# bioinformatics-centre/BayesTyper

Measured on AMD Instinct MI355X. Metric: variant-cluster Gibbs iterations/sec + k-mer matches/sec at 1/2/4/8 MI355X, higher is better.
Workload: dtype f64 log-probabilities over u8 k-mer counts (Gibbs); u64/u8 integer (k-mer matching)

## Files before the change

bayestyper_amd/csrc/bt_gibbs.hip:

```cpp
#ifndef BT_SWEEP_OUTLINE
#define BT_SWEEP_INLINE
#endif
#include "bt_gibbs_kernel.hpp"
#include "bt_internal.hpp"

#include <algorithm>
#include <atomic>
#include <chrono>
#include <cmath>
#include <cstring>
#include <map>
#include <memory>
#include <numeric>

using namespace bt;

namespace bt {
hipError_t launch_gibbs_simple_kernel(unsigned grid, uint32_t lds, hipStream_t st, const TileDesc *tiles, uint8_t *pool, const GParams *P, int op, uint32_t a0, uint32_t a1,
                                      unsigned long long *hist, TraceCfg tr, const uint32_t *tile_list);
hipError_t prepare_gibbs_simple_kernel(int max_lds);
hipError_t launch_gibbs_hot_kernel(unsigned grid, unsigned block, uint32_t lds, hipStream_t st, const TileDesc *tiles, uint8_t *pool, const GParams *P, int op, uint32_t a0, uint32_t a1,
                                   unsigned long long *hist, TraceCfg tr, const uint32_t *tile_list);
hipError_t prepare_gibbs_hot_kernel(int max_lds);
hipError_t occupancy_gibbs_hot_kernel(int *blocks_per_cu, int block, uint32_t lds);
// ... 664 lines not shown
    const bool fork = g->classes.size() > 1;
    if (fork) BT_HIP(hipEventRecord(g->ev_fork, g->ctx->stream));
    const char *order_env = getenv("BT_GIBBS_ORDER");
    const bool hot_first = order_env && std::strcmp(order_env, "hot_first") == 0 && (op == OP_RUN || op == OP_SWEEP);
    const bool ordered = (op == OP_RUN || op == OP_SWEEP) && !getenv("BT_GIBBS_UNORDERED_START");
    const bt_gibbs::LaunchClass *prev = nullptr;
    for (auto &c : g->classes) {
        hipStream_t st = c.stream ? c.stream : g->ctx->stream;
        if (c.stream) BT_HIP(hipStreamWaitEvent(st, g->ev_fork, 0));
        if (ordered && prev) BT_HIP(hipStreamWaitEvent(st, prev->ready, 0));
        if (hot_first && !c.stream)
            for (auto &o : g->classes)
                if (o.stream) BT_HIP(hipStreamWaitEvent(st, o.done, 0));
        if (op == OP_SWEEP && g->prefill_armed && c.num_prefill) {
            const unsigned threads = (uint64_t)c.num_prefill * g->S >= 4096 ? 64u : 256u;
            hipLaunchKernelGGL(ucache_prefill_kernel, dim3(c.num_prefill, g->S), dim3(threads), 0, st, (const TileDesc *)g->d_tiles, g->d_pool, (const GParams *)g->d_params,
                               (const PrefillItem *)c.d_prefill);
            BT_CHECK_LAUNCH();
        }
        if (ordered) {
            BT_HIP(hipEventRecord(c.ready, st));
            prev = &c;
        }
        if (op == OP_NOISE && (size_t)g->S * 1024 <= kHotBudget && !g->noise_in_gibbs_kernel) {
            const unsigned grid = (unsigned)std::min<size_t>(c.tiles.size(), (size_t)g->ctx->num_cu * 4);
            hipLaunchKernelGGL(gibbs_noise_kernel, dim3(grid), dim3(LANES * c.split), (size_t)g->S * 1024, st, (const TileDesc *)g->d_tiles, g->d_pool, (const GParams *)g->d_params, a0, hist,
                               (const uint32_t *)c.d_tiles, (uint32_t)c.tiles.size());
        } else if (c.simple && (op == OP_RUN || op == OP_SWEEP || op == OP_INIT_CHAIN))
            BT_HIP(launch_gibbs_simple_kernel((unsigned)c.tiles.size(), c.lds, st, g->d_tiles, g->d_pool, g->d_params, op, a0, a1, hist, tr, (const uint32_t *)c.d_tiles));
        else if (c.single && (op == OP_RUN || op == OP_SWEEP || op == OP_INIT_CHAIN))
            BT_HIP(launch_gibbs_single_kernel(c.pack_wgs, LANES * c.pack_waves, c.pack_lds, st, g->d_tiles, g->d_pool, g->d_params, op, a0, a1, hist, tr, (const uint32_t *)c.d_pack));
        else if (c.hot && (op == OP_RUN || op == OP_SWEEP || op == OP_INIT_CHAIN))
            BT_HIP(launch_gibbs_hot_kernel(c.pack_wgs, LANES * c.pack_waves, c.pack_lds, st, g->d_tiles, g->d_pool, g->d_params, op, a0, a1, hist, tr, (const uint32_t *)c.d_pack));
        else
            hipLaunchKernelGGL(gibbs_kernel, dim3((unsigned)c.tiles.size()), dim3(LANES * c.split), c.lds, st, g->d_tiles, g->d_pool, g->d_params, op, a0, a1, hist, tr,
                               (const uint32_t *)c.d_tiles);
        BT_CHECK_LAUNCH();
        if (wide && c.num_fill) {
            hipLaunchKernelGGL(nan_fill_kernel, dim3(c.num_fill), dim3(256), 0, st, g->d_pool, (const FillChunk *)c.d_fill);
            BT_CHECK_LAUNCH();
        }
        if (c.stream) BT_HIP(hipEventRecord(c.done, st));
    }
    for (auto &c : g->classes)
        if (c.stream) BT_HIP(hipStreamWaitEvent(g->ctx->stream, c.done, 0));
    g->prefill_armed = wide;
    return BT_OK;
}

inline uint64_t align_up(uint64_t x, uint64_t a) { return (x + a - 1) / a * a; }
inline uint32_t tile_lds_bytes(const TileDesc &d) { return d.lds_all ? d.hot_bytes * d.nvm : d.hot_bytes; }
constexpr uint32_t kMinTileWidth = 4;
constexpr uint32_t kLightLds = 24576;
const uint32_t kClassLds[] = {16384, 32768, 0xFFFFFFFFu};

const uint32_t kElemSize[A_COUNT] = {
     1,  1,  1,  1,  4,  4,  2,  4,  2,  4,  4,  4,  2,
     1,  4,  4,  4,  2,  4,  4,  4,  4,  4,  4,
     4,  1,
     4,  8,  8,  4,  4,  4,  4,  1,  2,  8,  4,  1,
     4,  4,  4,  4,  4,  4,  8,  4,  8,  2,  8,
     8,  4,  8,  1,  4,  4,  8,  1,  1,  8,  4,  8,  4,  1,  4,  8,  4,
     4,  1,  8,  4,  4,  4,  1,  1,  1,  1,  4,  2,  4,  8,  8,  4,  2,  1,  4,  4,  4,  1,  1,  1,  1,  4,  4};

}

extern "C" {

struct bt_gibbs_source {
    bt_ctx *ctx = nullptr;
    uint32_t S = 0, G = 0, C = 0;
    std::vector<ClusterDims> cd;
    std::vector<GroupDims> gd;
    BuildBatch dev{};
    std::vector<void *> allocs;
    uint64_t device_bytes = 0, flat_bytes = 0;
    bool uploaded = false;
};

static int validate_batch(const bt_gibbs_batch *B) {
    const uint32_t G = B->num_groups, C = B->num_clusters;
    if (G == 0 || C == 0) return fail("bt_gibbs_create: empty batch");
    if (B->group_cluster_off[G] != C) return fail("bt_gibbs_create: group_cluster_off[G] != num_clusters");
    {
        auto monotone = [](const uint32_t *off, uint64_t n) {
            for (uint64_t i = 0; i < n; ++i)
                if (off[i + 1] < off[i]) return false;
            return true;
        };
        if (B->group_cluster_off[0] != 0 || !monotone(B->group_cluster_off, G) || !monotone(B->group_source_off, G) || !monotone(B->edge_off, C) || !monotone(B->kmer_off, C) ||
            !monotone(B->unique_off, C) || !monotone(B->multi_off, C) || !monotone(B->nestdep_off, C) || !monotone(B->kv_off, B->kmer_off[C]) ||
            !monotone(B->nestdep_var_off, B->nestdep_off[C]))
            return fail("bt_gibbs_create: an offset array of the batch is not monotone");
        uint64_t hap_at = 0, var_at = 0, hv_at = 0;
        for (uint32_t gi = 0; gi < G; ++gi) {
            const uint32_t c0 = B->group_cluster_off[gi], c1 = B->group_cluster_off[gi + 1], nv = c1 - c0;
            if (nv == 0) return fail("bt_gibbs_create: group without clusters");
            for (uint32_t i = B->group_source_off[gi]; i < B->group_source_off[gi + 1]; ++i)
                if (B->group_sources[i] >= nv) return fail("bt_gibbs_create: source vertex outside its group");
            for (uint32_t c = c0; c < c1; ++c) {
                const uint32_t H = B->num_haplotypes[c], V = B->num_variants[c], K = B->kmer_off[c + 1] - B->kmer_off[c];
                for (uint32_t i = B->edge_off[c]; i < B->edge_off[c + 1]; ++i)
                    if (B->edges[i] >= nv) return fail("bt_gibbs_create: edge target outside its group");
                for (uint32_t i = B->unique_off[c]; i < B->unique_off[c + 1]; ++i)
                    if (B->unique_idx[i] >= K) return fail("bt_gibbs_create: unique k-mer index outside its cluster");
                for (uint32_t i = B->multi_off[c]; i < B->multi_off[c + 1]; ++i)
// ... 237 lines not shown
            return _rc;          \
        }                        \
    } while (0)
#define BT_TRYHIP(x)                                                     \
    do {                                                                 \
        hipError_t _e = (x);                                             \
        if (_e != hipSuccess) {                                          \
            bt_gibbs_destroy(g);                                         \
            return fail(std::string(#x) + ": " + hipGetErrorString(_e)); \
        }                                                                \
    } while (0)

    g->h_A.assign(C, 0);
    uint64_t flat_sel = 0;
    for (uint32_t c = 0; c < C; ++c) {
        g->h_A[c] = cd[c].A;
        flat_sel += (uint64_t)cd[c].K * cd[c].H + (uint64_t)cd[c].K * (S + 11ull) + (uint64_t)cd[c].nnz * (2 + 4 * ((cd[c].H + 31) / 32)) + ((uint64_t)cd[c].nu + cd[c].nm) * 4 +
                    (uint64_t)cd[c].H * cd[c].V * 2 + (uint64_t)cd[c].H * 4 + (uint64_t)cd[c].hn * 4;
    }

    const bool timing = getenv("BT_GIBBS_DEBUG") != nullptr;
    auto t_prev = std::chrono::steady_clock::now();
    std::string t_text;
    auto lap = [&](const char *what) {
        if (!timing) return;
        const auto now = std::chrono::steady_clock::now();
        char buf[96];
        snprintf(buf, sizeof buf, " %s %.1f ms;", what, std::chrono::duration<double, std::milli>(now - t_prev).count());
        t_text += buf;
        t_prev = now;
    };
    struct GShape {
        uint32_t nv, Hmax, Kmax, g;
    };
    std::vector<GShape> shapes(G);
    for (uint32_t gi = 0; gi < G; ++gi) {
        GShape s{gd[gi].nv, 0, 0, gi};
        for (uint32_t c = gd[gi].c0; c < gd[gi].c0 + gd[gi].nv; ++c) {
            s.Hmax = std::max(s.Hmax, cd[c].H);
            s.Kmax = std::max(s.Kmax, cd[c].K);
        }
        shapes[gi] = s;
    }
    std::stable_sort(shapes.begin(), shapes.end(), [](const GShape &a, const GShape &b) {
        if (a.nv != b.nv) return a.nv > b.nv;
        if (a.Hmax != b.Hmax) return a.Hmax > b.Hmax;
        return a.Kmax > b.Kmax;
    });
    std::vector<uint32_t> tile_start, blk_first, blk_last;
    std::vector<TilePlan> plans;
    uint64_t pool = 0;
    uint32_t ntiles = 0;
    uint32_t noise_level = 0;
    auto plan_tiles = [&](uint32_t relax) {
    tile_start.clear();
    pool = 0;
    const uint64_t dense_limit = relax >= 4 ? (64ull << 20) : (256ull << 20);
    {
        const uint32_t tail_h = getenv("BT_GIBBS_TAIL_H") ? (uint32_t)atoi(getenv("BT_GIBBS_TAIL_H")) : 16u;
        uint32_t n_x = 0;
        while (n_x < G && (shapes[n_x].nv > 1 || shapes[n_x].Hmax >= tail_h)) ++n_x;
        uint32_t n_y = n_x;
        while (n_y < G && shapes[n_y].Hmax >= 6) ++n_y;
        uint32_t width_x = kMinTileWidth, width_y = 16;
        const bool noise_widths = params->noise_seeding && !getenv("BT_GIBBS_NO_NOISE_WIDTHS");
        uint32_t width_z3 = LANES;
        if (noise_widths) {
            if (noise_level == 0) width_y = 8, width_z3 = 32;
            else if (noise_level == 1) width_y = 16, width_z3 = 32;
            else width_y = 16, width_z3 = LANES;
        }
        width_x = std::min<uint32_t>(LANES, width_x << relax);
        width_y = std::min<uint32_t>(LANES, width_y << relax);
        if (const char *e = getenv("BT_GIBBS_TAIL_WIDTH")) {
            const int v = atoi(e);
            if (v == 1 || v == 2 || v == 4 || v == 8 || v == 16 || v == 32 || v == 64) width_x = (uint32_t)v;
        }
        if (const char *e = getenv("BT_GIBBS_MID_WIDTH")) {
            const int v = atoi(e);
            if (v == 4 || v == 8 || v == 16 || v == 32 || v == 64) width_y = (uint32_t)v;
        }
        auto hashed = [&](uint32_t i) { return (uint64_t)S * ((uint64_t)shapes[i].Hmax * (shapes[i].Hmax + 1) / 2 + shapes[i].Hmax) > 65536; };
        uint32_t n_w = 0;
        for (uint32_t i = 0; i < n_x; ++i) n_w += hashed(i) ? 1u : 0u;
        uint32_t width_w = 1;
        while (width_w < width_x && (uint64_t)n_w > (uint64_t)width_w * (4 * 256)) width_w *= 2;
        if (const char *e = getenv("BT_GIBBS_HUGE_WIDTH")) {
            const int v = atoi(e);
            if (v == 1 || v == 2 || v == 4 || v == 8 || v == 16) width_w = (uint32_t)v;
        }
        width_w = std::min<uint32_t>(width_x, width_w << relax);
        uint32_t at = 0;
        while (at < n_x) {
            const bool hw = hashed(at);
            uint32_t run_end = at;
            while (run_end < n_x && hashed(run_end) == hw) ++run_end;
            const uint32_t w = hw ? width_w : width_x;
            while (at < run_end) {
                tile_start.push_back(at);
                at += std::min<uint32_t>(w, run_end - at);
            }
        }
        while (at < n_y) {
            tile_start.push_back(at);
            at += std::min<uint32_t>(width_y, n_y - at);
        }
        uint32_t n_z = n_y, n_z3 = n_y;
        if (noise_widths) {
            while (n_z < G && shapes[n_z].Hmax >= 4) ++n_z;
// ... 215 lines not shown
        for (int a = 0; a < A_COUNT; ++a) {
            off = align_up(off, 256);
            d.off[a] = off;
            off += len[a] * tile_w * kElemSize[a];
            if (a == A_PLOIDY) in_bytes = align_up(off, 256);
        }
        {
            for (int a = 0; a < A_COUNT; ++a) d.hoff[a] = NOHOT;
            const int hot_arrs[] = {A_SC, A_DIP, A_NESTPL, A_NESTN, A_KSCUPD, A_MGEN, A_PEND, A_PENDDIP, A_PENDVALID, A_EVN, A_FREQ, A_LOGF, A_OBS, A_NZ, A_NZLIST,
                                    A_UNEXT, A_ZHDR, A_ZBKT, A_PHDR, A_PBKT, A_KSCTMP, A_CUM, A_RING, A_FNDSAVED, A_UCACHE};
            d.lds_stride = 1;
            while (d.lds_stride < d.num_lanes) d.lds_stride *= 2;
            uint64_t ho = 0;
            bool want_simple = d.nvm == 1 && d.Hm == 2 && d.NMm == 0 && d.cache_mode == 0 && d.lds_stride == LANES && !getenv("BT_GIBBS_NO_SIMPLE") && !getenv("BT_GIBBS_NO_SIMPLE_KERNEL");
            for (uint32_t l = 0; l < d.num_lanes && want_simple; ++l) want_simple = cd[gd[shapes[tile_start[ti] + l].g].c0].H == 2;
            const uint64_t skip_mask = getenv("BT_GIBBS_HOT_SKIP") ? strtoull(getenv("BT_GIBBS_HOT_SKIP"), nullptr, 0) : 0ull;
            int hot_i = -1;
            for (int a : hot_arrs) {
                ++hot_i;
                if ((skip_mask >> hot_i) & 1ull) continue;
                if (a == A_MGEN && d.NMm == 0) continue;
                if (a == A_KSCTMP) continue;
                if (a == A_CUM && d.D2m * d.teams > 16) continue;
                if (want_simple && a != A_RING) continue;
                if (a == A_UCACHE && !(d.cache_mode == 0 && d.uc_width == 0 && d.nvm == 1 && (uint64_t)d.cache_entries * 8 <= 160)) continue;
                const uint64_t per_vertex = len[a] / nv;
                d.hoff[a] = (uint32_t)ho;
                ho = align_up(ho + per_vertex * d.lds_stride * kElemSize[a], 16);
            }
            d.sblk = 0;
            if (want_simple) {
                d.sblk = (uint32_t)ho;
                ho = align_up(ho + (uint64_t)3 * S * LANES * 4, 16);
            }
            d.hot_bytes = (uint32_t)std::min<uint64_t>(ho, 0xFFFFFFFFu);
            const uint64_t hot_budget = getenv("BT_GIBBS_HOT_BUDGET") ? strtoull(getenv("BT_GIBBS_HOT_BUDGET"), nullptr, 0) : kHotBudget;
            d.lds_all = d.nvm > 1 && ho * d.nvm <= hot_budget && !getenv("BT_GIBBS_NO_LDS_ALL") ? 1u : 0u;
            if (ho > hot_budget || (d.nvm > 1 && !d.lds_all && hot_budget < kHotBudget) || (d.nvm > 1 && getenv("BT_GIBBS_NOHOT_MULTI"))) {
                for (int a = 0; a < A_COUNT; ++a) d.hoff[a] = NOHOT;
                d.hot_bytes = 0;
                d.lds_all = 0;
            }
        }
        d.split = d.Hm < 6 ? 1u : (tile_lds_bytes(d) > kLightLds ? 2u : 4u);
        if (const char *e = getenv("BT_GIBBS_SPLIT")) {
            const int v = atoi(e);
            if (v == 1 || v == 2 || v == 4 || v == 8) d.split = (uint32_t)v;
        }
        d.copies = 1;
        if (d.lds_stride <= 32 && !getenv("BT_GIBBS_NO_COPIES")) {
            d.split = 1;
            d.copies = 64u / d.lds_stride;
        }
        {
            bool simple = d.nvm == 1 && d.Hm == 2 && d.NMm == 0 && d.cache_mode == 0 && d.copies == 1 && d.split == 1 && d.hot_bytes != 0 && !getenv("BT_GIBBS_NO_SIMPLE");
            for (uint32_t l = 0; l < d.num_lanes && simple; ++l) simple = cd[gd[shapes[tile_start[ti] + l].g].c0].H == 2;
            simple = simple && d.sblk != 0 && d.hoff[A_RING] != NOHOT && d.hoff[A_SC] == NOHOT;
            d.simple = simple ? 1u : 0u;
        }
        d.logged = d.nvm == 1 && d.NMm == 0 && !getenv("BT_GIBBS_NO_LOG") ? 1u : 0u;
        d.prio = (d.copies > 1 || d.num_lanes < LANES / 2) && !getenv("BT_GIBBS_NO_PRIO") ? 1u : 0u;
        d.base = ti == blk_first[ti] ? pool : plans[blk_first[ti]].d.base;
        if (ti == 0 && getenv("BT_GIBBS_DEBUG") && atoi(getenv("BT_GIBBS_DEBUG")) >= 2) {
            std::vector<std::pair<uint64_t, int>> by_size;
            for (int a = 0; a < A_COUNT; ++a) by_size.emplace_back(len[a] * tile_w * kElemSize[a], a);
            std::sort(by_size.rbegin(), by_size.rend());
            fprintf(stderr, "bt_gibbs: tile 0 (%u groups, %u vertices max, Hm %u, Km %u, S %u): %.1f MB;", d.num_lanes, d.nvm, d.Hm, d.Km, S, (double)align_up(off, 256) / 1048576.0);
            for (int i = 0; i < 6; ++i) fprintf(stderr, " array %d: %.1f MB", by_size[i].second, (double)by_size[i].first / 1048576.0);
            fprintf(stderr, "\n");
        }
        plans[ti].d = d;
        plans[ti].in_bytes = in_bytes;
        plans[ti].total_bytes = align_up(off, 256);
        if (ti == blk_first[ti]) pool += plans[ti].total_bytes;
    }
    };
    {
        size_t free_b = 0, total_b = 0;
        if (hipMemGetInfo(&free_b, &total_b) != hipSuccess) free_b = 0;
        for (uint32_t relax = 0;; ++relax) {
            plan_tiles(relax);
            if (relax >= 4 || free_b == 0 || pool + 256 <= (uint64_t)(0.92 * (double)free_b)) break;
        }
        while (params->noise_seeding && !getenv("BT_GIBBS_NO_NOISE_WIDTHS") && noise_level < 2) {
            uint32_t simple_need = 0;
            for (uint32_t ti = 0; ti < ntiles; ++ti)
                if (plans[ti].d.simple) simple_need = std::max(simple_need, tile_lds_bytes(plans[ti].d));
            const uint64_t per_cu = std::min<uint64_t>(8, 163840 / (((uint64_t)simple_need + 15) / 16 * 16 + (S * NC_BINS + 8u + NC_HELP_MAXH / 2u) * 4u));
            if ((uint64_t)ntiles <= per_cu * ctx->num_cu) break;
            ++noise_level;
            plan_tiles(0);
        }
    }
    lap("shape sort + tile plan");
    if (!plan_bytes)
        BT_TRYHIP(arena_reserve(ctx, (size_t)ntiles * (sizeof(TileDesc) + 64) + (size_t)C * (sizeof(BuildCluster) + sizeof(ClusterLoc) + 32) + (size_t)G * (sizeof(BuildGroup) + 16) + (8u << 20)));
    g->pool_bytes = pool + 256;
    if (plan_bytes) {
        const uint64_t flat = (uint64_t)C * 160 + (uint64_t)G * (32 + S) + flat_sel;
        *plan_bytes = g->pool_bytes + (uint64_t)S * (65536 + 256) * 8 + (uint64_t)ntiles * sizeof(TileDesc) + (uint64_t)C * sizeof(ClusterLoc) + flat;
        bt_gibbs_destroy(g);
        return BT_OK;
    }
    if (ctx->pool_cache && recycles && ctx->pool_cache_bytes >= g->pool_bytes && ctx->pool_cache_bytes / 2 <= g->pool_bytes + (64u << 20)) {
        g->d_pool = static_cast<uint8_t *>(ctx->pool_cache);
        g->pool_alloc_bytes = ctx->pool_cache_bytes;
        ctx->pool_cache = nullptr;
        ctx->pool_cache_bytes = 0;
// ... 391 lines not shown
            BT_TRYHIP(staged_upload(ctx, c.d_tiles, c.tiles.data(), c.tiles.size() * 4));
            std::vector<FillChunk> fill;
            for (uint32_t ti : c.tiles) {
                const TileDesc &d = g->tiles[ti];
                if (!(d.cache_mode == 0 && !d.simple && d.cache_entries > BT_UC_INVALIDATE_MIN && d.hoff[A_UCACHE] == NOHOT)) continue;
                const uint64_t words = ((uint64_t)d.nvm * d.cache_entries) << d.wsh;
                for (uint64_t w = 0; w < words; w += 32768) fill.push_back(FillChunk{d.base + d.off[A_UCACHE] + w * 8, (uint32_t)std::min<uint64_t>(32768, words - w), 0u});
            }
            std::vector<PrefillItem> pre;
            if (!fill.empty() && !getenv("BT_GIBBS_NO_PREFILL")) {
                std::vector<uint8_t> in_class(ntiles, 0);
                for (uint32_t ti : c.tiles) {
                    const TileDesc &d = g->tiles[ti];
                    in_class[ti] = d.cache_mode == 0 && !d.simple && d.cache_entries > BT_UC_INVALIDATE_MIN && d.hoff[A_UCACHE] == NOHOT;
                }
                for (uint32_t gi = 0; gi < g->G; ++gi)
                    if (in_class[g->group_tile[gi]])
                        for (uint32_t v = 0; v < g->group_nvert[gi]; ++v) pre.push_back(PrefillItem{g->group_tile[gi], g->group_lane[gi], v, 0u});
            }
            if (!pre.empty()) {
                BT_TRYHIP(hipMalloc(reinterpret_cast<void **>(&c.d_prefill), pre.size() * sizeof(PrefillItem)));
                g->allocs.push_back(c.d_prefill);
                BT_TRYHIP(staged_upload(ctx, c.d_prefill, pre.data(), pre.size() * sizeof(PrefillItem)));
                c.num_prefill = (uint32_t)pre.size();
            }
            if (!fill.empty() && !getenv("BT_GIBBS_NO_WIDE_FILL")) {
                BT_TRYHIP(hipMalloc(reinterpret_cast<void **>(&c.d_fill), fill.size() * sizeof(FillChunk)));
                g->allocs.push_back(c.d_fill);
                BT_TRYHIP(staged_upload(ctx, c.d_fill, fill.data(), fill.size() * sizeof(FillChunk)));
                c.num_fill = (uint32_t)fill.size();
            }
            lap("class lists");
            BT_TRYHIP(hipEventCreateWithFlags(&c.ready, hipEventDisableTiming));
            if (i + 1 < g->classes.size()) {
                int prio_lo = 0, prio_hi = 0;
                BT_TRYHIP(hipDeviceGetStreamPriorityRange(&prio_lo, &prio_hi));
                int prio = getenv("BT_GIBBS_NO_PRIO") ? prio_lo : prio_hi;
                if (const char *e = getenv("BT_GIBBS_CLASS_PRIO")) prio = atoi(e);
                BT_TRYHIP(ctx_class_streams(ctx, (unsigned)i + 1, prio, class_streams));
                c.stream = class_streams[i];
                BT_TRYHIP(hipEventCreateWithFlags(&c.done, hipEventDisableTiming));
            }
            lap("class stream");
        }
        if (getenv("BT_GIBBS_DEBUG")) {
            std::vector<uint32_t> bins(40, 0);
            for (uint32_t ti = 0; ti < ntiles; ++ti) bins[std::min<uint32_t>(39, tile_lds_bytes(g->tiles[ti]) / 2048)] += 1;
            fprintf(stderr, "bt_gibbs: tiles by LDS need:");
            for (uint32_t b = 0; b < 40; ++b)
                if (bins[b]) fprintf(stderr, " [%u-%u KB: %u]", 2 * b, 2 * b + 2, bins[b]);
            fprintf(stderr, "\n");
        }
        if (getenv("BT_GIBBS_DEBUG")) {
            fprintf(stderr, "bt_gibbs: %u tiles in %zu launch classes:", ntiles, g->classes.size());
            for (auto &c : g->classes) fprintf(stderr, " [%zu tiles, lds %u B, split %u%s%s]", c.tiles.size(), c.lds, c.split, c.simple ? ", simple" : "", c.single ? ", single" : (c.hot ? ", hot" : ""));
            fprintf(stderr, "; tile 0: hot_bytes %u lds_stride %u copies %u\n", g->tiles[0].hot_bytes, g->tiles[0].lds_stride, g->tiles[0].copies);
            for (size_t i = 0; i < g->classes.size(); ++i) {
                const auto &c = g->classes[i];
                std::map<std::string, uint32_t> setups;
                for (uint32_t ti : c.tiles) {
                    const TileDesc &d = g->tiles[ti];
                    const bool inval = d.cache_mode == 0 && d.cache_entries > BT_UC_INVALIDATE_MIN;
                    const bool wide = inval && !d.simple && d.hoff[A_UCACHE] == NOHOT;
                    char buf[256];
                    snprintf(buf, sizeof buf, "Hm=%u nvm=%u NMm=%u lanes=%u cache_mode=%u entries=%u table=%s teams=%u copies=%u scache_n=%u", d.Hm, d.nvm, d.NMm, d.num_lanes,
                             d.cache_mode, d.cache_entries, d.cache_mode ? "tagged" : (wide ? "wide" : (inval ? "invalidated" : "whole")), d.teams, d.copies, d.scache_n);
                    setups[buf] += 1;
                }
                fprintf(stderr, "bt_gibbs: class %zu kernel=%s:", i, c.simple ? "simple" : (c.single ? "single" : (c.hot ? "hot" : "generic")));
                for (auto &s : setups) fprintf(stderr, " [%s tiles=%u]", s.first.c_str(), s.second);
                fprintf(stderr, "\n");
            }
        }
    }
    BT_TRYHIP(hipStreamSynchronize(ctx->stream));
    lap("tables, launch classes");
    BT_TRY(launch(g, OP_SETUP, 0, 0, nullptr));
    BT_TRYHIP(hipStreamSynchronize(ctx->stream));
#undef BT_TRY
#undef BT_TRYHIP
    lap("set-up launch (synchronised)");
    if (timing) fprintf(stderr, "bt_gibbs: construction of %u groups in %u tiles, pool %.1f MB:%s\n", G, ntiles, g->pool_bytes / 1048576.0, t_text.c_str());
    *out = g;
    return BT_OK;
}

int bt_gibbs_destroy(bt_gibbs *g) {
    if (!g) return BT_OK;
    (void)hipSetDevice(g->ctx->device);
    if (g->nc.active) (void)bt_gibbs_noise_chain_end(g);
    (void)hipStreamSynchronize(g->ctx->stream);
    const bool dbg_release = getenv("BT_GIBBS_DEBUG") != nullptr;
    const auto t_rel0 = std::chrono::steady_clock::now();
    for (void *p : g->allocs) {
        if (!p) continue;
        if (p == g->d_pool && g->keep_pool && !g->ctx->pool_cache && g->pool_alloc_bytes) {
            g->ctx->pool_cache = p;
            g->ctx->pool_cache_bytes = g->pool_alloc_bytes;
            continue;
        }
        (void)hipFree(p);
    }
    const auto t_rel1 = std::chrono::steady_clock::now();
    if (g->d_trace) (void)hipFree(g->d_trace);
    if (g->d_trace_counter) (void)hipFree(g->d_trace_counter);
    if (g->d_wire) (void)hipFree(g->d_wire);
// ... 868 lines not shown
```

bayestyper_amd/csrc/bt_gibbs_tile.hpp:

```cpp
#pragma once
#include "bt_rng_device.hpp"

namespace bt {

constexpr unsigned LANES = 64;
constexpr uint16_t NOHAP = 0xFFFF;
constexpr double BT_LN2 = 0.693147180559945309417232121458176568;
constexpr double BT_DBL_EPS = 2.220446049250313080847263336181640625e-16;
#ifndef BT_LINEAR_DRAW_MIN
#define BT_LINEAR_DRAW_MIN 4u
#endif
#ifndef BT_UC_INVALIDATE_MIN
#define BT_UC_INVALIDATE_MIN 64u
#endif
#ifndef BT_EVAL_BLOCK
#define BT_EVAL_BLOCK 4u
#endif
constexpr uint32_t EVB = BT_EVAL_BLOCK;
#ifdef BT_SINGLE
constexpr bool kSingle = true;
#else
constexpr bool kSingle = false;
#endif
#ifdef BT_PACKED
// ... 58 lines not shown
    A_SCLEN,
    A_KSC,
    A_KSCUPD,
    A_DIPKEYS,
    A_DIPFREQ,
    A_ASTATS,
    A_NESTPL, A_NESTN,
    A_NESTST,
    A_KSCKEY,
    A_KSCDATA,
    A_EVLOG,
    A_EVN,
    A_NVER,
    A_PENDNEST,
    A_SC,
    A_EDGES,
    A_COVER,
    A_MCACHE,
    A_MCTAG,
    A_MCGEN,
    A_MGEN,
    A_OTH,
    A_SUBM,
    A_SUBCNT,
    A_SUBIC,
    A_SKVOFF,
    A_SKVVAR,
    A_SKVBITS,
    A_KSCTMP,
    A_LOGF,
    A_PEND,
    A_PENDDIP,
    A_PENDVALID,
    A_SOURCES,
    A_STACK,
    A_BRNG,
    A_SHMULT,
    A_MSUBM,
    A_MSUBC,
    A_MSUBIC,
    A_MSUBSH,
    A_RING,
    A_COUNT
};

struct TileDesc {
    uint32_t S, nvm, Hm, Vm, Km, HWm, NUm, NMm, NNZm, HNm, NDm, NDVm, NEm, NSHm, Am, Bcap, D2m, Dcm, cache_mode, cache_entries, dip_cap, scache_n, scache_len,
        scache_p, num_lanes, first_group;
    uint64_t base;
    uint64_t trace_base;
    uint64_t off[A_COUNT];
    uint32_t hoff[A_COUNT];
    uint32_t hot_bytes, split;
    uint32_t copies, copies_pad;
    uint32_t uc_width;
    uint32_t mat_width;
    uint32_t lds_stride, lds_all;
    uint32_t simple;
    uint32_t ring_cap[2], ring_len;
    uint32_t prio;
    uint32_t pool_lane0;
    uint32_t logged;
    uint32_t wsh;
    uint32_t teams;
    uint32_t sblk;
};
#ifndef BT_EV_CAP
#define BT_EV_CAP 32
#endif
constexpr uint32_t EV_CAP = BT_EV_CAP;
constexpr uint32_t KSC_WAYS = 4;
constexpr uint32_t KSC_NOKEY = 0xFFFEFFFEu;
constexpr uint32_t NOHOT = 0xFFFFFFFFu;
constexpr uint32_t RESIDENT_ALL = 0xFFFFFFFEu;
constexpr uint32_t RESIDENT_NEVER = 0xFFFFFFFDu;

struct GParams {
    uint32_t S, seed, num_chains, burn_in, num_iterations, max_hvk, noise_seeding;
    double rate;
    uint8_t gender[32];
    const double BT_GAS *lut_g;
    const double BT_GAS *lut_n;
    const double BT_GAS *lgamma_int;
    const double BT_GAS *gamma_a2;
    uint32_t lgamma_n, gamma_n;
};

extern __shared__ __attribute__((aligned(16))) uint8_t bt_lds_raw[];
__device__ inline uint8_t *lds_block() { return (uint8_t *)bt_lds_raw; }
__device__ inline uint32_t pack_slot() { return blockIdx.x * (blockDim.x >> 6) + (uint32_t)__builtin_amdgcn_readfirstlane((int)(threadIdx.x >> 6)); }

__host__ __device__ constexpr bool hot_core(int a) {
    return a == A_SC || a == A_DIP || a == A_NESTPL || a == A_NESTN || a == A_KSCUPD || a == A_PEND || a == A_PENDDIP || a == A_PENDVALID || a == A_EVN || a == A_FREQ || a == A_LOGF ||
           a == A_OBS || a == A_NZ || a == A_NZLIST || a == A_UNEXT || a == A_ZHDR || a == A_ZBKT || a == A_PHDR || a == A_PBKT || a == A_RING || a == A_FNDSAVED;
}

struct Tile {
    uint8_t BT_GAS *base;
    const TileDesc BT_CAS *d;
    uint32_t lane;
    uint32_t plane;
    uint32_t part, copies;
    uint32_t wsh;
    uint8_t *hot;
    uint32_t lds0;
    uint32_t resident;
    template <typename T>
// ... 53 lines not shown
    __device__ inline uint8_t M(uint32_t k, uint32_t h) const { return mat(A_M, d().Km)[(uint32_t)k * d().Hm + h]; }
    __device__ inline uint8_t has_counts(uint32_t k) const { return a<uint8_t>(A_HASC, d().Km)[k]; }
    __device__ inline uint8_t count(uint32_t k, uint32_t s) const { return a<uint8_t>(A_COUNTS, (uint32_t)d().Km * d().S)[(uint32_t)k * d().S + s]; }
    __device__ inline uint8_t ic(uint32_t k, uint32_t g) const { return a<uint8_t>(A_IC, (uint32_t)d().Km * 2)[2 * k + g]; }
    __device__ inline int32_t shared_idx(uint32_t k) const { return a<int32_t>(A_SHARED, d().Km)[k]; }
    __device__ inline uint32_t kv_off(uint32_t k) const { return a<uint32_t>(A_KVOFF, d().Km + 1)[k]; }
    __device__ inline uint16_t kv_var(uint32_t e) const { return a<uint16_t>(A_KVVAR, d().NNZm)[e]; }
    __device__ inline bool kv_bit(uint32_t e, uint32_t h) const { return (a<uint32_t>(A_KVBITS, (uint32_t)d().NNZm * d().HWm)[(uint32_t)e * d().HWm + (h >> 5)] >> (h & 31u)) & 1u; }
    __device__ inline uint32_t hap_cell(uint32_t h, uint32_t var) const { return a<uint32_t>(A_HAPCELL, (uint32_t)d().Hm * d().Vm)[(uint32_t)h * d().Vm + var]; }
    __device__ inline TPtr<double> astats_cell(uint32_t s, uint32_t cell) const { return a<double>(A_ASTATS, (uint32_t)d().S * d().Am * 12) + ((uint32_t)s * d().Am + cell) * 12; }
    __device__ inline uint16_t hap_allele(uint32_t h, uint32_t var) const { return a<uint16_t>(A_HAPAL, (uint32_t)d().Hm * d().Vm)[(uint32_t)h * d().Vm + var]; }
    __device__ inline uint32_t hn_off(uint32_t h) const { return a<uint32_t>(A_HNOFF, d().Hm + 1)[h]; }
    __device__ inline uint32_t hn_idx(uint32_t i) const { return a<uint32_t>(A_HNIDX, d().HNm)[i]; }
    __device__ inline uint16_t var_na(uint32_t var) const { return a<uint16_t>(A_VARNA, d().Vm)[var]; }
    __device__ inline uint8_t var_dep(uint32_t var) const { return a<uint8_t>(A_VARDEP, d().Vm)[var]; }
    __device__ inline uint32_t allele_base(uint32_t var) const { return a<uint32_t>(A_ALBASE, d().Vm + 1)[var]; }
    __device__ inline uint32_t *mt(uint32_t g) const { return (uint32_t *)(t.base + d().off[A_MT]) + ((size_t)((v * 2 + g) << t.wsh) + t.plane) * MT_RING_PAD; }
    __device__ inline SPtrF<uint32_t, LANES> ring(uint32_t g) const { return t.harr<uint32_t>(A_RING, v, d().ring_len) + (g ? d().ring_cap[0] + MT_RING_HDR : 0u); }
    __device__ inline MtRing rng(uint32_t g) const { return mt_ring_open(mt(g), ring(g), d().ring_cap[g]); }
    __device__ inline void rng_seed(uint32_t g, uint32_t seed) const { mt_ring_seed(mt(g), ring(g), d().ring_cap[g], seed); }
    __device__ inline SPtrF<uint32_t, LANES> sc() const { return t.harr<uint32_t>(A_SC, v, SC_COUNT); }
    __device__ inline TPtr<uint32_t> uniq() const { return a<uint32_t>(A_UNIQ, d().NUm); }
    __device__ inline TPtr<uint32_t> multi() const { return a<uint32_t>(A_MULTI, d().NMm); }
    __device__ inline TPtr<uint32_t> usub() const { return a<uint32_t>(A_USUB, d().NUm); }
    __device__ inline TPtr<uint32_t> msub() const { return a<uint32_t>(A_MSUB, d().NMm); }
    __device__ inline TPtr<uint8_t> smm() const { return a<uint8_t>(A_SMM, (uint32_t)d().NMm * d().S); }
    __device__ inline SPtrF<uint16_t, LANES> dip() const { return t.harr<uint16_t>(A_DIP, v, 2 * d().S); }
    __device__ inline SPtrF<double, LANES> freq() const { return t.harr<double>(A_FREQ, v, d().Hm); }
    __device__ inline RPtr<uint8_t> subm() const { return mat(A_SUBM, d().NUm); }
    __device__ inline TPtr<uint8_t> subcnt() const { return a<uint8_t>(A_SUBCNT, d().NUm * d().S); }
    __device__ inline TPtr<uint8_t> subic() const { return a<uint8_t>(A_SUBIC, d().NUm * 2); }
    __device__ inline TPtr<uint32_t> skv_off() const { return a<uint32_t>(A_SKVOFF, d().NUm + 1); }
    __device__ inline TPtr<uint16_t> skv_var() const { return a<uint16_t>(A_SKVVAR, d().NNZm > 1 ? d().NNZm : 1); }
    __device__ inline TPtr<uint32_t> skv_bits() const { return a<uint32_t>(A_SKVBITS, (d().NNZm > 1 ? d().NNZm : 1) * d().HWm); }
    __device__ inline SPtrF<double, LANES> ksc_tmp() const { return t.harr<double>(A_KSCTMP, v, 2 * d().Vm * 4); }
    __device__ inline SPtrF<double, LANES> logf() const { return t.harr<double>(A_LOGF, v, d().Hm); }
    __device__ inline SPtrF<uint32_t, LANES> obs() const { return t.harr<uint32_t>(A_OBS, v, d().Hm); }
    __device__ inline SPtrF<uint8_t, LANES> nz() const { return t.harr<uint8_t>(A_NZ, v, d().Hm); }
    __device__ inline SPtrF<uint32_t, LANES> unext() const { return t.harr<uint32_t>(A_UNEXT, v, d().Hm); }
    typedef USetP<SPtrF<uint32_t, LANES>> HSet;
    __device__ inline HSet zero_set() const { return HSet{t.harr<uint32_t>(A_ZHDR, v, 4), t.harr<uint32_t>(A_ZBKT, v, d().Bcap), unext(), d().Bcap}; }
    __device__ inline HSet plus_set() const { return HSet{t.harr<uint32_t>(A_PHDR, v, 4), t.harr<uint32_t>(A_PBKT, v, d().Bcap), unext(), d().Bcap}; }
    __device__ inline TPtr<uint32_t> hvcount() const { return a<uint32_t>(A_HVCOUNT, (uint32_t)d().Hm * d().Vm); }
    __device__ inline UCPtr ucache() const {
        const uint32_t ho = d().hoff[A_UCACHE];
        if (t.hot != nullptr && ho != NOHOT && (t.resident == RESIDENT_ALL || v == t.resident))
            return UCPtr{(double *)(t.hot + (t.resident == RESIDENT_ALL ? v * d().hot_bytes : 0u) + ho), t.lane, t.wsh};
        double *b = (double *)(uint8_t *)(t.base + d().off[A_UCACHE]);
        const uint32_t w = d().uc_width;
        if (w) return UCPtr{b, (v * w + t.plane) * d().cache_entries, 0u};
        return UCPtr{b, ((v * d().cache_entries) << t.wsh) + t.plane, t.wsh};
    }
    __device__ inline TPtr<uint32_t> uctag() const { return a<uint32_t>(A_UCTAG, d().cache_mode == 1 ? d().cache_entries : 1); }
    __device__ inline SPtrF<double, LANES> cum() const { return t.harr<double>(A_CUM, v, (d().D2m > 1 ? d().D2m : 1) * (d().teams > 1 ? d().teams : 1)); }
    __device__ inline SPtrF<uint16_t, LANES> nzlist() const { return t.harr<uint16_t>(A_NZLIST, v, d().Hm); }
    __device__ inline TPtr<double> simplex() const { return a<double>(A_SIMPLEX, d().Hm + 1); }
    __device__ inline TPtr<double> scache() const { return a<double>(A_SCACHE, (uint32_t)(d().scache_n ? d().scache_n : 1) * (d().scache_len ? d().scache_len : 1)); }
    __device__ inline TPtr<uint32_t> sclen() const { return a<uint32_t>(A_SCLEN, d().scache_n > 1 ? d().scache_n : 1); }
    __device__ inline TPtr<double> ksc(uint32_t s, uint32_t which, uint32_t var) const {
        return a<double>(A_KSC, (uint32_t)d().S * 2 * d().Vm * 4) + (((uint32_t)s * 2 + which) * d().Vm + var) * 4;
    }
    __device__ inline SPtrF<uint8_t, LANES> ksc_upd() const { return t.harr<uint8_t>(A_KSCUPD, v, d().S); }
    __device__ inline TPtr<uint32_t> dip_keys() const { return a<uint32_t>(A_DIPKEYS, d().dip_cap); }
    __device__ inline TPtr<uint32_t> dip_freq() const { return a<uint32_t>(A_DIPFREQ, (uint32_t)d().dip_cap * d().S); }
    __device__ inline TPtr<double> astats(uint32_t s, uint32_t var, uint32_t al) const {
        return a<double>(A_ASTATS, (uint32_t)d().S * d().Am * 12) + ((uint32_t)s * d().Am + allele_base(var) + al) * 12;
    }
    __device__ inline SPtrF<uint8_t, LANES> nest_ploidy() const { return t.harr<uint8_t>(A_NESTPL, v, d().S); }
    __device__ inline SPtrF<uint8_t, LANES> nest_n() const { return t.harr<uint8_t>(A_NESTN, v, d().S); }
    __device__ inline TPtr<uint32_t> ksc_key(uint32_t s) const { return a<uint32_t>(A_KSCKEY, (uint32_t)d().S * (KSC_WAYS + 1u)) + (uint32_t)s * (KSC_WAYS + 1u); }
    __device__ inline TPtr<double> ksc_data(uint32_t s, uint32_t e) const {
        return a<double>(A_KSCDATA, (uint32_t)d().S * KSC_WAYS * 2 * d().Vm * 4) + ((uint32_t)s * KSC_WAYS + e) * 2 * d().Vm * 4;
    }
    __device__ inline TPtr<uint32_t> evlog(uint32_t s) const { return a<uint32_t>(A_EVLOG, (uint32_t)d().S * (2u * EV_CAP + 1u)) + (uint32_t)s * (2u * EV_CAP + 1u); }
    __device__ inline SPtrF<uint8_t, LANES> evn() const { return t.harr<uint8_t>(A_EVN, v, d().S); }
    __device__ inline TPtr<uint32_t> nver() const { return a<uint32_t>(A_NVER, (uint32_t)d().S * 2); }
    __device__ inline TPtr<double> pend_nest(uint32_t s) const { return a<double>(A_PENDNEST, (uint32_t)d().S * 8) + (uint32_t)s * 8; }
    __device__ inline TPtr<double> nest_stats(uint32_t s, uint32_t j) const { return a<double>(A_NESTST, (uint32_t)d().S * 8) + ((uint32_t)s * 2 + j) * 4; }
    __device__ inline TPtr<uint32_t> edges() const { return a<uint32_t>(A_EDGES, d().NEm > 1 ? d().NEm : 1); }
    __device__ inline TPtr<uint8_t> cover_rows() const { return a<uint8_t>(A_COVER, d().Km); }
    __device__ inline TPtr<double> mcache() const { return a<double>(A_MCACHE, d().cache_entries); }
    __device__ inline TPtr<uint32_t> mctag() const { return a<uint32_t>(A_MCTAG, d().cache_entries); }
    __device__ inline TPtr<uint32_t> mcgen() const { return a<uint32_t>(A_MCGEN, d().cache_entries); }
    __device__ inline SPtrF<uint32_t, LANES> mgen() const { return t.harr<uint32_t>(A_MGEN, v, d().S); }
    __device__ inline TPtr<uint8_t> oth() const { return a<uint8_t>(A_OTH, d().NMm * d().S); }
    __device__ inline TPtr<uint8_t> msubm() const { return a<uint8_t>(A_MSUBM, (d().NMm > 1 ? d().NMm : 1) * d().Hm); }
    __device__ inline TPtr<uint8_t> msubc() const { return a<uint8_t>(A_MSUBC, (d().NMm > 1 ? d().NMm : 1) * d().S); }
    __device__ inline TPtr<uint8_t> msubic() const { return a<uint8_t>(A_MSUBIC, (d().NMm > 1 ? d().NMm : 1) * 2); }
    __device__ inline TPtr<uint32_t> msubsh() const { return a<uint32_t>(A_MSUBSH, d().NMm > 1 ? d().NMm : 1); }
    __device__ inline SPtrF<uint32_t, LANES> pend() const { return t.harr<uint32_t>(A_PEND, v, d().S); }
    __device__ inline SPtrF<uint16_t, LANES> pend_dip() const { return t.harr<uint16_t>(A_PENDDIP, v, 2 * d().S); }
    __device__ inline SPtrF<uint8_t, LANES> pend_valid() const { return t.harr<uint8_t>(A_PENDVALID, v, d().S); }
    __device__ inline double &fnd_saved() const { return t.harr<double>(A_FNDSAVED, v, 1)[0]; }
    __device__ inline double BT_GAS &sparsity() const { return a<double>(A_SPARSITY, 1)[0]; }
    __device__ inline NormalState fnd() const { return NormalState{&fnd_saved(), &sc()[SC_FND_AVAIL]}; }
    __device__ inline TPtr<uint8_t> shared_mult() const { return t.arr<uint8_t>(A_SHMULT); }
};

__device__ inline uint32_t tile_split(const TileDesc BT_CAS *d) {
    if (kPacked) return 1u;
    const uint32_t waves = blockDim.x >> 6;
    return d->split < waves ? d->split : waves;
}
__device__ inline uint32_t tile_lane(uint32_t split, uint32_t copies) { return (kPacked ? 0u : (threadIdx.x >> 6) * (64u / split)) + ((threadIdx.x & 63u) % (64u / copies)); }
__device__ inline uint32_t tile_part(uint32_t copies) { return (threadIdx.x & 63u) / (64u / copies); }
__device__ inline bool tile_thread_active(uint32_t split, uint32_t copies) {
    if (kPacked) return true;
// ... 1155 lines not shown
                        TPtr<double> q = c.nest_stats(s, j);
                        same = same && (double)q[0] == (double)pn[4 * j] && (double)q[1] == (double)pn[4 * j + 1] && (double)q[2] == (double)pn[4 * j + 2];
                    }
            } else
                same = true;
            if (same) {
                c.pend()[s] += 1;
                continue;
            }
        }
#endif
#ifdef BT_COLLECT_OUTLINE
        collect_sample_slow(env, vtx, s);
#else
        collect_sample_body(c, P, s, nsub_u, nsub_m);
#endif
    }
}

__device__ BT_SWEEPFN void sample_diplotypes(Env env, uint32_t vtx, bool collect, uint32_t trace_word, bool tracing, uint32_t *trace_buf) {
    const Vx c = make_vx(make_tile(env), vtx);
    const GParams BT_CAS &P = env_params(env);
    const TPtr<uint32_t> trace_row{(uint32_t BT_GAS *)uniform_ptr(trace_buf), trace_word, 6u};
    SPtrF<uint32_t, LANES> sc = c.sc();
    const uint32_t nsub_u = sc[SC_NSUB_U], nsub_m = kSingle ? 0u : (uint32_t)sc[SC_NSUB_M];
    const bool use_multi = !kSingle && sc[SC_USE_MULTI] != 0, is_sparse = sc[SC_IS_SPARSE] != 0;
    uint32_t hap_count = sc[SC_HAP_COUNT];
    PROF_DECL;
    if (sc[SC_UC_DIRTY] == 2u) {
        const Vx::UCPtr ucl = c.ucache();
        const double nan = __builtin_nan("");
        for (uint32_t i = c.t.part, n = c.d().cache_entries; i < n; i += c.t.copies) ucl[i] = nan;
        if (c.t.copies > 1u) copies_sync();
        sc[SC_UC_DIRTY] = 0;
    } else if (sc[SC_UC_DIRTY]) {
        fill_unique_cache(env, vtx);
        sc[SC_UC_DIRTY] = 0;
    }
    PROF(12);
    MtRing rng = c.rng(0);
    SPtrF<uint16_t, LANES> nzl = c.nzlist();
    SPtrF<double, LANES> logf = c.logf();
    SPtrF<uint16_t, LANES> dip = c.dip();
    uint32_t nnz = 0;
    {
        SPtrF<uint8_t, LANES> nz = c.nz();
        for (uint32_t h = 0; h < c.H; ++h)
            if (nz[h]) nzl[nnz++] = (uint16_t)h;
    }
    PROF(0);
    const uint32_t T = c.t.copies > 1u && c.d().teams > 1u ? c.d().teams : 1u;
    const uint32_t tsz = c.t.copies / T, team = c.t.part / tsz, tpart = c.t.part - team * tsz;
    const uint32_t cw = 64u / c.t.copies, gl = (threadIdx.x & 63u) % cw, tlane0 = gl + team * tsz * cw;
    SPtrF<double, LANES> cum = c.cum() + (team < T ? team : 0u) * (c.d().D2m > 1 ? c.d().D2m : 1);
    for (uint32_t s0 = 0; s0 < P.S; s0 += T) {
      double u01 = 0;
      for (uint32_t j = 0; j < T && s0 + j < P.S; ++j) {
          const double u = rng_canonical(rng);
          if (j == team) u01 = u;
      }
      PROF(24);
      const uint32_t s = s0 + team;
      uint32_t mine = 0xFFFFFFFFu;
      if (team < T && s < P.S) {
        const uint16_t p1 = dip[2 * s], p2 = dip[2 * s + 1];
        const uint8_t ploidy = c.nest_ploidy()[s];
        uint32_t gen = 0;
        if (use_multi && nsub_m) {
            multi_refresh(c, P, s, p1, p2, nsub_m);
            gen = c.mgen()[s];
        }
        PROF(1);
        const uint32_t total = ploidy == 2 ? nnz * (nnz + 1) / 2 : (ploidy == 1 ? nnz : 0u);
        const bool chain_only = total <= BT_LINEAR_DRAW_MIN;
        const bool par = !chain_only && tsz > 1u;
        double lpmax = 0;
        auto eval_candidates = [&]() {
            const bool dipl = ploidy == 2;
            const TileDesc BT_CAS &dd = c.d();
            const Vx::UCPtr uc = c.ucache();
            TPtr<double> mc = c.mcache();
            TPtr<uint32_t> uct = c.uctag(), mct = c.mctag(), mcg = c.mcgen();
            const bool multi = use_multi && nsub_m != 0;
            uint32_t a = 0, b = 0;
            auto advance = [&](uint32_t steps) {
                if (!dipl) {
                    a += steps;
                    return;
                }
                while (steps > 0 && a < nnz) {
                    const uint32_t left = nnz - b;
                    if (steps < left) {
                        b += steps;
                        steps = 0;
                    } else {
                        steps -= left;
                        ++a;
                        b = a;
                    }
                }
            };
            const uint32_t stride_blocks = par ? tsz : 1u;
            if (par) advance(EVB * tpart);
            lpmax = -__builtin_huge_val();
            for (uint32_t base = par ? EVB * tpart : 0u; base < total; base += EVB * stride_blocks) {
                const uint32_t nb = total - base < EVB ? total - base : EVB;
                uint16_t ha[EVB], hb[EVB];
// ... 376 lines not shown
```

Measured before the change: 1.206 billion.

## Place cumulative scratch and unique-sum cache in spare LDS without losing occupancy

Adds an occupancy-aware LDS budget per tile. A binary search through the HIP occupancy API finds the largest dynamic LDS size that keeps the current blocks-per-CU, and the freed room is used to make the cumulative-probability scratch resident in LDS, either whole or as a prefix window, and to hold the unique-sum cache when it fits. The device-side cum accessor now returns a split pointer that reads LDS below the window and global memory above it, so every access pays an extra branch. The new plan is skipped when noise seeding is on, and it also raises the kernels' maximum dynamic LDS attribute.

```diff
diff --git a/bayestyper_amd/csrc/bt_gibbs.hip b/bayestyper_amd/csrc/bt_gibbs.hip
--- a/bayestyper_amd/csrc/bt_gibbs.hip
+++ b/bayestyper_amd/csrc/bt_gibbs.hip
@@ -740,6 +740,8 @@
 inline uint32_t tile_lds_bytes(const TileDesc &d) { return d.lds_all ? d.hot_bytes * d.nvm : d.hot_bytes; }
 constexpr uint32_t kMinTileWidth = 4;
 constexpr uint32_t kLightLds = 24576;
+constexpr uint32_t kResidencyCapDefault = 0xFFFFFFFFu;
+constexpr uint32_t kCumWindowMin = 10;
 const uint32_t kClassLds[] = {16384, 32768, 0xFFFFFFFFu};
 
 const uint32_t kElemSize[A_COUNT] = {
@@ -1083,9 +1085,46 @@
     uint64_t pool = 0;
     uint32_t ntiles = 0;
     uint32_t noise_level = 0;
+    const bool residency_legacy = params->noise_seeding != 0 || (getenv("BT_GIBBS_RESIDENCY") && !strcmp(getenv("BT_GIBBS_RESIDENCY"), "legacy"));
+    const uint32_t residency_cap_bound = getenv("BT_GIBBS_LDS_CAP") ? (uint32_t)strtoul(getenv("BT_GIBBS_LDS_CAP"), nullptr, 0) : kResidencyCapDefault;
+    struct ResidencyStats {
+        uint32_t cum_full = 0, cum_window = 0, cum_window_min = 0xFFFFFFFFu, cum_window_max = 0, ucache = 0;
+        uint64_t legacy_bytes = 0, bytes = 0;
+    } rstats;
+    std::map<std::pair<int, int>, uint32_t> cap_memo;
+    auto residency_cap = [&](bool hot_kind, uint32_t need) -> uint32_t {
+        auto occ = [&](uint32_t lds, int *o) {
+            *o = 0;
+            const hipError_t e = hot_kind ? occupancy_gibbs_hot_kernel(o, (int)LANES, lds)
+                                          : hipOccupancyMaxActiveBlocksPerMultiprocessor(o, reinterpret_cast<const void *>(gibbs_kernel), (int)LANES, lds);
+            if (e != hipSuccess) (void)hipGetLastError();
+            return e == hipSuccess && *o > 0;
+        };
+        int o0 = 0;
+        if (need >= kHotBudget || !occ(need, &o0)) return need;
+        const auto key = std::make_pair(hot_kind ? 1 : 0, o0);
+        const auto hit = cap_memo.find(key);
+        if (hit != cap_memo.end()) return std::max(hit->second, need);
+        uint32_t lo = need / 256, hi = kHotBudget / 256;
+        while (lo < hi) {
+            const uint32_t mid = (lo + hi + 1) / 2;
+            int o = 0;
+            if (occ(mid * 256, &o) && o >= o0) lo = mid;
+            else hi = mid - 1;
+        }
+        const uint32_t cap = std::max(lo * 256, need);
+        cap_memo[key] = lo * 256;
+        return cap;
+    };
+    if (!residency_legacy) {
+        (void)prepare_gibbs_hot_kernel((int)kHotBudget);
+        (void)hipFuncSetAttribute(reinterpret_cast<const void *>(gibbs_kernel), hipFuncAttributeMaxDynamicSharedMemorySize, (int)kHotBudget);
+        (void)hipGetLastError();
+    }
     auto plan_tiles = [&](uint32_t relax) {
     tile_start.clear();
     pool = 0;
+    rstats = ResidencyStats{};
     const uint64_t dense_limit = relax >= 4 ? (64ull << 20) : (256ull << 20);
     {
         const uint32_t tail_h = getenv("BT_GIBBS_TAIL_H") ? (uint32_t)atoi(getenv("BT_GIBBS_TAIL_H")) : 16u;
@@ -1407,8 +1446,44 @@
             d.split = 1;
             d.copies = 64u / d.lds_stride;
         }
+        if (d.hot_bytes != 0 && d.sblk == 0) {
+            const uint32_t legacy_need = tile_lds_bytes(d);
+            const uint64_t skip_mask = getenv("BT_GIBBS_HOT_SKIP") ? strtoull(getenv("BT_GIBBS_HOT_SKIP"), nullptr, 0) : 0ull;
+            if (d.hoff[A_CUM] != NOHOT) d.cum_win = std::max<uint32_t>(d.D2m, 1);
+            if (!residency_legacy && d.split == 1) {
+                bool hot_kind = !getenv("BT_GIBBS_NO_HOT_KERNEL") && (d.nvm == 1 || d.lds_all);
+                for (int a = 0; a < A_COUNT && hot_kind; ++a)
+                    if (hot_core(a)) hot_kind = d.hoff[a] != NOHOT;
+                const uint32_t nvert = d.lds_all ? d.nvm : 1u;
+                const uint64_t cap = std::min<uint64_t>(std::min<uint32_t>(residency_cap(hot_kind, legacy_need), residency_cap_bound), kHotBudget);
+                uint64_t ho = d.hot_bytes;
+                auto room = [&]() { return cap / nvert > ho ? cap / nvert - ho : 0ull; };
+                if (d.hoff[A_CUM] == NOHOT && !((skip_mask >> 21) & 1ull)) {
+                    const uint32_t D2 = std::max<uint32_t>(d.D2m, 1);
+                    const uint64_t per_entry = (uint64_t)d.teams * d.lds_stride * 8;
+                    const uint32_t win = (uint32_t)std::min<uint64_t>(D2, room() / per_entry);
+                    if (win >= std::min<uint32_t>(D2, kCumWindowMin)) {
+                        d.hoff[A_CUM] = (uint32_t)ho;
+                        d.cum_win = win;
+                        ho = align_up(ho + win * per_entry, 16);
+                        (win == D2 ? rstats.cum_full : rstats.cum_window) += 1;
+                        if (win < D2) rstats.cum_window_min = std::min(rstats.cum_window_min, win), rstats.cum_window_max = std::max(rstats.cum_window_max, win);
+                    }
+                }
+                if (d.hoff[A_UCACHE] == NOHOT && !((skip_mask >> 24) & 1ull) && d.cache_mode == 0 && d.cache_entries <= BT_UC_INVALIDATE_MIN && (d.nvm == 1 || d.lds_all) &&
+                    (uint64_t)d.cache_entries * d.lds_stride * 8 <= room()) {
+                    d.hoff[A_UCACHE] = (uint32_t)ho;
+                    d.uc_width = 0;
+                    ho = align_up(ho + (uint64_t)d.cache_entries * d.lds_stride * 8, 16);
+                    rstats.ucache += 1;
+                }
+                d.hot_bytes = (uint32_t)ho;
+            }
+            rstats.legacy_bytes += legacy_need;
+            rstats.bytes += tile_lds_bytes(d);
+        }
         {
-            bool simple = d.nvm == 1 && d.Hm == 2 && d.NMm == 0 && d.cache_mode == 0 && d.copies == 1 && d.split == 1 && d.hot_bytes != 0 && !getenv("BT_GIBBS_NO_SIMPLE");
+            bool simple =d.nvm == 1 && d.Hm == 2 && d.NMm == 0 && d.cache_mode == 0 && d.copies == 1 && d.split == 1 && d.hot_bytes != 0 && !getenv("BT_GIBBS_NO_SIMPLE");
             for (uint32_t l = 0; l < d.num_lanes && simple; ++l) simple = cd[gd[shapes[tile_start[ti] + l].g].c0].H == 2;
             simple = simple && d.sblk != 0 && d.hoff[A_RING] != NOHOT && d.hoff[A_SC] == NOHOT;
             d.simple = simple ? 1u : 0u;
@@ -1906,6 +1981,14 @@
             fprintf(stderr, "\n");
         }
         if (getenv("BT_GIBBS_DEBUG")) {
+            uint64_t charged = 0;
+            for (auto &c : g->classes)
+                if (!c.simple) charged += (uint64_t)c.tiles.size() * c.lds;
+            fprintf(stderr, "bt_gibbs: residency plan=%s cap_bound=%u: candidate scratch resident whole in %u more tiles, as a window in %u (%u to %u entries), unique sums in %u more; lds_need=%llu legacy_need=%llu charged=%llu\n",
+                    residency_legacy ? "legacy" : "budget", residency_cap_bound, rstats.cum_full, rstats.cum_window, rstats.cum_window ? rstats.cum_window_min : 0u, rstats.cum_window_max, rstats.ucache, (unsigned long long)rstats.bytes,
+                    (unsigned long long)rstats.legacy_bytes, (unsigned long long)charged);
+        }
+        if (getenv("BT_GIBBS_DEBUG")) {
             fprintf(stderr, "bt_gibbs: %u tiles in %zu launch classes:", ntiles, g->classes.size());
             for (auto &c : g->classes) fprintf(stderr, " [%zu tiles, lds %u B, split %u%s%s]", c.tiles.size(), c.lds, c.split, c.simple ? ", simple" : "", c.single ? ", single" : (c.hot ? ", hot" : ""));
             fprintf(stderr, "; tile 0: hot_bytes %u lds_stride %u copies %u\n", g->tiles[0].hot_bytes, g->tiles[0].lds_stride, g->tiles[0].copies);
diff --git a/bayestyper_amd/csrc/bt_gibbs_tile.hpp b/bayestyper_amd/csrc/bt_gibbs_tile.hpp
--- a/bayestyper_amd/csrc/bt_gibbs_tile.hpp
+++ b/bayestyper_amd/csrc/bt_gibbs_tile.hpp
@@ -134,7 +134,8 @@
     uint64_t off[A_COUNT];
     uint32_t hoff[A_COUNT];
     uint32_t hot_bytes, split;
-    uint32_t copies, copies_pad;
+    uint32_t copies;
+    uint32_t cum_win;
     uint32_t uc_width;
     uint32_t mat_width;
     uint32_t lds_stride, lds_all;
@@ -294,7 +295,21 @@
         return UCPtr{b, ((v * d().cache_entries) << t.wsh) + t.plane, t.wsh};
     }
     __device__ inline TPtr<uint32_t> uctag() const { return a<uint32_t>(A_UCTAG, d().cache_mode == 1 ? d().cache_entries : 1); }
-    __device__ inline SPtrF<double, LANES> cum() const { return t.harr<double>(A_CUM, v, (d().D2m > 1 ? d().D2m : 1) * (d().teams > 1 ? d().teams : 1)); }
+    struct CumPtr {
+        SPtrF<double, LANES> lds, mem;
+        uint32_t win;
+        __device__ inline double &operator[](uint32_t i) const { return i < win ? lds[i] : mem[i]; }
+    };
+    __device__ inline CumPtr cum(uint32_t team) const {
+        const uint32_t D2 = d().D2m > 1 ? d().D2m : 1, T = d().teams > 1 ? d().teams : 1;
+        const SPtrF<double, LANES> mem{(double *)(uint8_t *)(t.base + d().off[A_CUM]), ((v * D2 * T + team * D2) << t.wsh) + t.plane, t.wsh};
+        const uint32_t ho = d().hoff[A_CUM];
+        if (t.hot != nullptr && ho != NOHOT && (t.resident == RESIDENT_ALL || v == t.resident)) {
+            const uint32_t win = d().cum_win;
+            return CumPtr{SPtrF<double, LANES>{(double *)(t.hot + (t.resident == RESIDENT_ALL ? v * d().hot_bytes : 0u) + ho), ((team * win) << t.wsh) + t.lane, t.wsh}, mem, win};
+        }
+        return CumPtr{mem, mem, 0u};
+    }
     __device__ inline SPtrF<uint16_t, LANES> nzlist() const { return t.harr<uint16_t>(A_NZLIST, v, d().Hm); }
     __device__ inline TPtr<double> simplex() const { return a<double>(A_SIMPLEX, d().Hm + 1); }
     __device__ inline TPtr<double> scache() const { return a<double>(A_SCACHE, (uint32_t)(d().scache_n ? d().scache_n : 1) * (d().scache_len ? d().scache_len : 1)); }
@@ -1556,7 +1571,7 @@
     const uint32_t T = c.t.copies > 1u && c.d().teams > 1u ? c.d().teams : 1u;
     const uint32_t tsz = c.t.copies / T, team = c.t.part / tsz, tpart = c.t.part - team * tsz;
     const uint32_t cw = 64u / c.t.copies, gl = (threadIdx.x & 63u) % cw, tlane0 = gl + team * tsz * cw;
-    SPtrF<double, LANES> cum = c.cum() + (team < T ? team : 0u) * (c.d().D2m > 1 ? c.d().D2m : 1);
+    const Vx::CumPtr cum = c.cum(team < T ? team : 0u);
     for (uint32_t s0 = 0; s0 < P.S; s0 += T) {
       double u01 = 0;
       for (uint32_t j = 0; j < T && s0 + j < P.S; ++j) {
```

Result: slower. 1.122 billion (-6.9%).
